# arpg/Kangaroo

Hardware: AMD Instinct MI355X
Metric: kinectfusion_frames_per_sec_640x480_to_512cubed_tsdf (higher is better)
Workload: dtype f32

## Files before the change

### include/kfx_debug.h

```cpp
#ifndef KFX_DEBUG_H
#define KFX_DEBUG_H

#include "kfx.h"

#ifdef __cplusplus
extern "C" {
#endif

int kfx_debug_rmw(const kfx_volume* vol, int variant, kfx_stream stream);

int kfx_debug_div_uniform_check(float b, unsigned long long* d_out, kfx_stream stream);

int kfx_debug_div_core_check(unsigned seed, int per_divisor, unsigned long long* d_out, kfx_stream stream);
int kfx_debug_sqrt_core_check(unsigned long long* d_out, kfx_stream stream);
int kfx_debug_wave_xor_check(unsigned seed, unsigned long long* d_out, kfx_stream stream);

int kfx_debug_summary_export(kfx_sdf_summary* s, float tol, float vref, int fine_shift, void* R_out, void* C_out, int dims_out[12],
                             kfx_stream stream);

int kfx_debug_summary_conditional_builds(kfx_sdf_summary* s, int out[2], kfx_stream stream);

int kfx_debug_summary_top_levels(kfx_sdf_summary* s, int fine_shift, void* top_out, int dims_out[12], unsigned long long* launches_out,
                                 kfx_stream stream);

int kfx_debug_fuse_keep(const kfx_sdf_summary* s, int out[3], unsigned char* kept, int n_rows);

#ifdef __cplusplus
}
#endif
#endif
```

### kangaroo_amd/csrc/raycast.hip

```cpp
#include <cmath>
#include <thread>

#include <hip/hip_fp16.h>

#include "kfx_device.h"
#include "sampling.h"
#include "raycast_ray.h"
#include "../../include/kfx_slab_color.h"

namespace kfx {

template <typename CELL, bool COLOR>
__device__ __forceinline__ void write_ray(const RayParams& q, const ColorGeom& cv, const int u, const int v, const float depth)
{
    const auto gradient_at = [&q](const V3 pos_w) { return gradient<CELL>(q, pos_w); };
    if constexpr (COLOR) write_ray(q, u, v, depth, gradient_at, [&cv](const V3 pos_w) { return trilinear<RayC32>(cv, pos_w); });
    else write_ray(q, u, v, depth, gradient_at, PhongShade{});
}

__device__ __forceinline__ unsigned touch(unsigned* bitmap, const VolView& v, int x, int y, int z)
{
    const size_t i = ((size_t)z * v.h + y) * v.w + x;
    const unsigned bit = 1u << (i & 31);
    unsigned* word = bitmap + (i >> 5);
    if (*reinterpret_cast<volatile unsigned*>(word) & bit) return 0u;
    return (atomicOr(word, bit) & bit) ? 0u : 1u;
}
__device__ __forceinline__ void touch_sample(unsigned* bitmap, const VolView& vol, const CellPos c, unsigned* cnt)
{
    cnt[0] += 1;
    for (int k = 0; k < 8; ++k) cnt[3] += touch(bitmap, vol, c.ix + (k & 1), c.iy + ((k >> 1) & 1), c.iz + (k >> 2));
}
__device__ __forceinline__ void touch_gradient(unsigned* bitmap, const RayParams& p, const V3 pos_w, unsigned* cnt)
{
    cnt[2] += 1;
    const CellPos b = gradient_base(p, pos_w);
    for (int dz = -1; dz < 2; ++dz)
        for (int dy = -1; dy < 2; ++dy)
            for (int dx = -1; dx < 2; ++dx)
                if ((dx < 0) + (dy < 0) + (dz < 0) <= 1) cnt[3] += touch(bitmap, p.vol, b.ix + dx, b.iy + dy, b.iz + dz);
}
// ... 12 lines not shown
}

template <typename CELL, bool COLOR, bool COUNT = false>
__device__ __forceinline__ float raycast_pixel(const RayParams& p, const ColorGeom& cv, const int u, const int v, unsigned* bitmap = nullptr,
                                               unsigned* cnt = nullptr)
{
    if (u >= p.w || v >= p.h) return 0.f;

    const RayBox box = ray_box(p, u, v);
    float depth = 0.0f;
    if (enters(box))
        depth = march_plain(p, box, [=](const RayParams& q, const V3 pos_w) {
            if constexpr (COUNT) touch_sample(bitmap, q.vol, cell_of(q, pos_w), cnt);
            return trilinear<CELL>(q, pos_w);
        });

    if constexpr (COUNT) {
        if (depth > 0) touch_gradient(bitmap, p, box.c_w + box.ray_w * depth, cnt);
    } else {
        write_ray<CELL, COLOR>(p, cv, u, v, depth);
    }
    return depth > 0 ? depth : __builtin_nanf("");
}

struct TopLevels { ClassLevel lv[2]; int n; };

__device__ __forceinline__ int class_lookup(const unsigned* tab, const ClassLevel& L, int gx, int gy, int gz)
{
    const int bx = gx >> L.shift, by = gy >> L.shift, bz = gz >> L.shift;
    const uint2 w = *reinterpret_cast<const uint2*>(tab + L.first + (bz * L.ny + by) * L.rw + ((bx >> 5) << 1));
    return (int)((w.x >> (bx & 31)) & 1u) | (int)(((w.y >> (bx & 31)) & 1u) << 1);
}

template <typename CELL, bool COLOR, bool COUNT = false, bool GT = false>
__device__ __forceinline__ float raycast_pixel_classes(const RayParams& p, const RayParams& q, const ColorGeom& cv, const int u, const int v, const ClassView& cl_arg, const unsigned* tab,
                                                       const TopLevels& top, unsigned* bitmap = nullptr, unsigned* cnt = nullptr)
{
    constexpr bool PARK = !GT && !COUNT;
    ClassView parked;
    if constexpr (PARK) parked = cl_arg;
    ClassView& clp = parked;
    if constexpr (PARK) {
        clp.fine.shift = in_vgpr(clp.fine.shift); clp.fine.ny = in_vgpr(clp.fine.ny); clp.fine.rw = in_vgpr(clp.fine.rw); clp.fine.first = in_vgpr(clp.fine.first);
        clp.coarse.ny = in_vgpr(clp.coarse.ny); clp.coarse.rw = in_vgpr(clp.coarse.rw); clp.coarse.first = in_vgpr(clp.coarse.first);
        clp.ox = in_vgpr(clp.ox); clp.oy = in_vgpr(clp.oy); clp.oz = in_vgpr(clp.oz);
        clp.eps = in_vgpr(clp.eps); clp.vref = in_vgpr(clp.vref);
    }
    const ClassView& cl = PARK ? parked : cl_arg;
    if (u >= p.w || v >= p.h) return 0.f;

    const RayBox box = ray_box(p, u, v);
    const V3 c_w = box.c_w, ray_w = box.ray_w;
    const float max_tmin = box.max_tmin, min_tmax = box.min_tmax;

    float depth = 0.0f;
    if (max_tmin < min_tmax) {
        float lambda = max_tmin;
        float last_sdf = __builtin_nanf("");
        const float min_delta = p.voxel.x;
        float delta = 0.f;
        const V3 sc = v3(p.dims1.x / p.size.x, p.dims1.y / p.size.y, p.dims1.z / p.size.z);
        const V3 pfA = v3((c_w.x - p.vol.bmin.x) * sc.x, (c_w.y - p.vol.bmin.y) * sc.y, (c_w.z - p.vol.bmin.z) * sc.z);
        const V3 pfB = v3(ray_w.x * sc.x, ray_w.y * sc.y, ray_w.z * sc.z);
        const V3 inv = v3(1.0f / pfB.x, 1.0f / pfB.y, 1.0f / pfB.z);
        const float eps = cl.eps;
        const float step_free = fmaxf(cl.vref, min_delta);
        const float inv_step_free = 1.0f / step_free, inv_trunc = 1.0f / p.trunc;
        const float band = cl.tol * cl.vref;
        bool pending = false;
        float lambda_prev = 0.f;
        bool consult = true;
        float lam_retry = lambda;
        int wait = 0, backoff = 1;
        while (lambda < min_tmax) {
            const bool look = consult && wait == 0 && lambda >= lam_retry;
            CellPos c{};
            typename CELL::InFlight fl;
            if (!look) {
                c = cell_of(p, c_w + ray_w * lambda);
                trilinear_issue<CELL>(fl, p, c);
                if constexpr (COUNT) touch_sample(bitmap, p.vol, c, cnt);
            }
            if (look) {
                if constexpr (COUNT) cnt[1] += 1;
                const float ex = __builtin_fmaf(pfB.x, lambda, pfA.x), ey = __builtin_fmaf(pfB.y, lambda, pfA.y), ez = __builtin_fmaf(pfB.z, lambda, pfA.z);
                const float flx = floorf(ex), fly = floorf(ey), flz = floorf(ez);
                const float lo_f = fminf(fminf(ex - flx, ey - fly), ez - flz), hi_f = fmaxf(fmaxf(ex - flx, ey - fly), ez - flz);
                bool run = false;
                if (fminf(fminf(ex, ey), ez) > eps && ex < p.dims1.x - eps && ey < p.dims1.y - eps && ez < p.dims1.z - eps && lo_f > eps && hi_f < 1.0f - eps) {
                    const int gx = (int)flx + cl.ox, gy = (int)fly + cl.oy, gz = (int)flz + cl.oz;
                    int cls = 0, shift = cl.fine.shift;
                    if constexpr (GT) {
                        if (cl.top_n > 1) {
                            int c7 = class_lookup(tab, top.lv[1], gx, gy, gz);
                            if (c7 == 3 && !cl.amb_ok) c7 = 0;
                            if (c7 != 0) { cls = c7; shift = 7; }
                        }
                        if (cls == 0 && cl.top_n > 0) {
                            int c6 = class_lookup(tab, top.lv[0], gx, gy, gz);
                            if (c6 == 3 && !cl.amb_ok) c6 = 0;
                            if (c6 != 0) { cls = c6; shift = 6; }
                        }
                        if (cls == 0) {
                            int c5 = class_lookup(cl.C, cl.coarse, gx, gy, gz);
                            if (c5 == 3 && !cl.amb_ok) c5 = 0;
                            if (c5 != 0) { cls = c5; shift = 5; }
                        }
                        if (cls == 0) {
// ... 46 lines not shown
                        backoff = 1;
                        run = true;
                    } else {
                        lam_retry = lam_exit;
                    }
                }
                if (!run) {
                    wait = backoff;
                    backoff = min(backoff * 2, 32);
                }
            }
            if (!look) {
                const float sdf = trilinear_finish<CELL>(fl, c);
                wait = max(wait - 1, 0);
                if (sdf <= 0) {
                    if (pending) {
                        last_sdf = trilinear<CELL>(p, c_w + ray_w * lambda_prev);
                        if constexpr (COUNT) touch_sample(bitmap, p.vol, cell_of(p, c_w + ray_w * lambda_prev), cnt);
                    }
                    if (last_sdf > 0) {
                        if (p.subpix) lambda = lambda + delta * sdf / (last_sdf - sdf);
                        depth = lambda;
                    }
                    break;
                }
                delta = march_step(sdf, min_delta, p.trunc);
                lambda += delta;
                last_sdf = sdf;
                pending = false;
                consult = !(fabsf(sdf - cl.vref) > band);
            }
        }
    }

    if constexpr (COUNT) {
        if (depth > 0) touch_gradient(bitmap, p, c_w + ray_w * depth, cnt);
    } else {
        write_ray<CELL, COLOR>(q, cv, u, v, depth);
    }
    return depth > 0 ? depth : __builtin_nanf("");
}

template <bool GT = false>
__device__ __forceinline__ void classes_stage(const ClassView& cl, unsigned* tab, TopLevels& top)
{
    const uint4* src = reinterpret_cast<const uint4*>(cl.C + (GT ? cl.top_first : 0));
    uint4* dst = reinterpret_cast<uint4*>(tab);
    for (int i = threadIdx.x; i < (cl.lds_words >> 2); i += blockDim.x) dst[i] = src[i];
    ClassLevel l6, l7;
    int nx6, nz6, nx7, nz7, w6, w7;
    const int at = GT ? 0 : cl.words;
    class_level_up(cl.nx5, cl.coarse.ny, cl.nz5, 6, at, l6, nx6, nz6, w6);
    class_level_up(nx6, l6.ny, nz6, 7, at + w6, l7, nx7, nz7, w7);
    if (threadIdx.x == 0) { top.lv[0] = l6; top.lv[1] = l7; top.n = cl.top_n; }
    __syncthreads();
}

__device__ __forceinline__ bool workgroup_any(const bool yes, int* s_any)
{
    const bool wave_any = __ballot(yes) != 0ull;
    if ((threadIdx.x & 63) == 0) s_any[threadIdx.x >> 6] = wave_any ? 1 : 0;
    __syncthreads();
    return (s_any[0] | s_any[1] | s_any[2] | s_any[3]) != 0;
}

template <typename CELL, bool GT = false>
__global__ __launch_bounds__(256) void k_raycast_sdf_classes(const RayParams p, const ClassView cl)
{
    extern __shared__ unsigned s_tab[];
    __shared__ RayParams s_p;
    __shared__ TopLevels s_top;
    __shared__ int s_any[4];
    if (threadIdx.x == 0) s_p = p;
    int u, v;
    const bool carries = ray_lane_pixel(p, p.sparse_lanes, blockIdx.x, blockIdx.y, u, v);
    const bool pixel = carries && u < p.w && v < p.h;
    if constexpr (!GT) {
        if (!workgroup_any(pixel && enters(ray_box(p, u, v)), s_any)) {
            if (pixel) write_no_hit(ray_out(p, u, v));
            return;
        }
    }
    classes_stage<GT>(cl, s_tab, s_top);
    if (!carries) return;
    raycast_pixel_classes<CELL, false, false, GT>(p, s_p, ColorGeom{}, u, v, cl, s_tab, s_top);
}

template <typename CELL, bool COLOR>
__global__ __launch_bounds__(256) void k_raycast_sdf(const RayParams p, const ColorGeom cv)
{
    int u, v;
    if (!ray_lane_pixel(p, p.sparse_lanes, blockIdx.x, blockIdx.y, u, v)) return;
    raycast_pixel<CELL, COLOR>(p, cv, u, v);
}

template <typename CELL>
__global__ __launch_bounds__(256) void k_raycast_sdf_count(const RayParams p, unsigned* __restrict__ bitmap, unsigned long long* __restrict__ counters)
{
    int u, v;
    ray_pixel_of(p, blockIdx.x, blockIdx.y, threadIdx.x, u, v);
    unsigned cnt[4] = {0u, 0u, 0u, 0u}, entered = 0;
    if (u < p.w && v < p.h) {
        entered = enters(ray_box(p, u, v)) ? 1u : 0u;
        raycast_pixel<CELL, false, true>(p, ColorGeom{}, u, v, bitmap, cnt);
    }
    publish_counts(cnt, entered, counters);
}

template <typename CELL, bool GT = false>
__global__ __launch_bounds__(256) void k_raycast_sdf_classes_count(const RayParams p, const ClassView cl, unsigned* __restrict__ bitmap,
                                                                   unsigned long long* __restrict__ counters)
{
    extern __shared__ unsigned s_tab[];
    __shared__ RayParams s_p;
    __shared__ TopLevels s_top;
    if (threadIdx.x == 0) s_p = p;
    classes_stage<GT>(cl, s_tab, s_top);
    int u, v;
    ray_pixel_of(p, blockIdx.x, blockIdx.y, threadIdx.x, u, v);
// ... 348 lines not shown
    cl.vref = vref;
    cl.amb_ok = fmaxf(vref, p.voxel.x) == p.trunc ? 1 : 0;
    cl.tol = tol;
    const double u24 = 1.0 / 16777216.0;
    double eps = 0.0;
    const float bmin[3] = {p.vol.bmin.x, p.vol.bmin.y, p.vol.bmin.z}, bmax[3] = {p.vol.bmax.x, p.vol.bmax.y, p.vol.bmax.z};
    const float size[3] = {p.size.x, p.size.y, p.size.z}, dims1[3] = {p.dims1.x, p.dims1.y, p.dims1.z};
    const float cw[3] = {p.T.m[3], p.T.m[7], p.T.m[11]};
    for (int a = 0; a < 3; ++a) {
        if (!(size[a] > 0.f)) return 0;
        const double sc = (double)dims1[a] / size[a];
        const double pmax = std::fmax(std::fabs((double)bmin[a]), std::fabs((double)bmax[a])), ca = std::fabs((double)cw[a]);
        const double A = std::fabs(((double)cw[a] - bmin[a]) * sc);
        const double t = sc * (3.0 * pmax + 2.0 * ca + size[a]) * u24 + 2.0 * dims1[a] * u24;
        const double e = u24 * (3.0 * A + 2.0 * sc * (pmax + ca) + dims1[a]) + 3.0 * u24 * (dims1[a] + A);
        eps = std::fmax(eps, t + e);
    }
    eps *= 2.0;
    if (!(eps < 0.05)) return 0;
    cl.eps = (float)std::fmax(eps, 1e-4);
    *lds_bytes = (size_t)cl.lds_words * sizeof(unsigned);
    *usable = 1;
    return 0;
}

template <typename PLAIN, typename... A>
static int launch_march(const char* what, int usable, const ClassView& cl, size_t cl_bytes, dim3 grid, kfx_stream stream, const RayParams& p,
                        void (*global)(RayParams, ClassView, A...), void (*lds)(RayParams, ClassView, A...), PLAIN plain, A... a)
{
    if (usable) hipLaunchKernelGGL(cl.global ? global : lds, grid, dim3(256), cl_bytes, (hipStream_t)stream, p, cl, a...);
    else plain();
    return check_launch(what);
}

template <typename CELL>
static int raycast_levels_launch(int n_levels, const kfx_image* const* depth, const kfx_image* const* norm, const kfx_image* const* img,
                                 const kfx_image* const* vbo, const kfx_volume* vol, const float T_wc[12], const float* K, float near, float far,
                                 float trunc_dist, int subpix, kfx_stream stream, kfx_sdf_summary* summary = nullptr)
{
    if (n_levels < 0 || n_levels > RAY_MAX_LEVELS) return set_error(KFX_E_RANGE, "RaycastSdf(levels): number of levels");
    if (!depth || !norm || !img || !K) return set_error(KFX_E_NULL, "RaycastSdf(levels): null argument");
    RayParams base{};
    RayLevels L{};
    int blocks = 0;
    for (int l = 0; l < n_levels; ++l) {
        RayParams p;
        if (int e = ray_params<CELL>(p, depth[l], norm[l], img[l], vol, T_wc, K + 4 * l, near, far, trunc_dist, subpix)) return e;
        if (p.w == 0 || p.h == 0) continue;
        RayLevel& lv = L.lv[L.n++];
        lv.dptr = p.dptr; lv.nptr = p.nptr; lv.iptr = p.iptr;
        lv.dpitch = p.dpitch; lv.npitch = p.npitch; lv.ipitch = p.ipitch;
        lv.w = p.w; lv.h = p.h;
        lv.K = p.K;
        lv.vptr = nullptr;
        lv.vpitch = 0;
        if (vbo && vbo[l]) {
            const kfx_image* vb = vbo[l];
            if (int e = check_image(vb, 16, (size_t)p.w, (size_t)p.h, "RaycastSdf(levels): vertex map")) return e;
            lv.vptr = (unsigned char*)vb->ptr;
            lv.vpitch = vb->pitch;
        }
        lv.first_block = blocks;
        static const int sparse_env = [] { const int v = env_int("KFX_RAYCAST_SPARSE", 16); return (v == 8 || v == 16 || v == 32) ? v : 0; }();
        lv.sparse = (long long)p.w * p.h <= 160 * 120 ? sparse_env : 0;
        lv.blocks_x = lv.sparse ? ceil_div(p.w, 2 * lv.sparse) : ceil_div(p.w, 64);
        blocks += lv.blocks_x * (lv.sparse ? ceil_div(p.h, 2) : ceil_div(p.h, 4));
// ... 9 lines not shown
        if (int e = class_view<CELL>(cl, &cl_bytes, &usable, summary, vol, base, stream, false)) return e;
        if (usable) {
            hipLaunchKernelGGL((k_raycast_sdf_levels_classes<CELL>), dim3(blocks), dim3(256), cl_bytes, (hipStream_t)stream, base, L, cl);
            return check_launch("kfx_raycast_sdf_levels_tracked");
        }
    }
    hipLaunchKernelGGL((k_raycast_sdf_levels<CELL>), dim3(blocks), dim3(256), 0, (hipStream_t)stream, base, L);
    return check_launch("kfx_raycast_sdf_levels");
}

template <typename CELL>
static int raycast_launch(const kfx_image* depth, const kfx_image* norm, const kfx_image* img,
                          const kfx_volume* vol, const float T_wc[12], const float K[4], float near,
                          float far, float trunc_dist, int subpix, kfx_stream stream, const kfx_volume* colorvol = nullptr,
                          kfx_sdf_summary* summary = nullptr)
{
    RayParams p;
    if (int e = ray_params<CELL>(p, depth, norm, img, vol, T_wc, K, near, far, trunc_dist, subpix)) return e;
    if (summary && summary->cell_bytes != CELL::BYTES)
        return set_error(KFX_E_SHAPE, "RaycastSdf(tracked): the summary was created for the other cell type (kfx_sdf_summary_create / _create_h)");
    if (p.w == 0 || p.h == 0) return 0;

    const dim3 grid = ray_tiling(p);
    ColorGeom cv{};
    if (colorvol) {
        if (int e = check_volume(colorvol, 4, 2, VOLUME_ANY_DIM, "RaycastSdf(colour)")) return e;
        set_geometry(cv, colorvol);
        hipLaunchKernelGGL((k_raycast_sdf<CELL, true>), grid, dim3(256), 0, (hipStream_t)stream, p, cv);
    } else if (summary) {
        ClassView cl;
        size_t cl_bytes = 0;
        int usable = 0;
        if (int e = class_view<CELL>(cl, &cl_bytes, &usable, summary, vol, p, stream)) return e;
        return launch_march("kfx_raycast_sdf_tracked", usable, cl, cl_bytes, grid, stream, p, k_raycast_sdf_classes<CELL, true>, k_raycast_sdf_classes<CELL, false>,
                            [&] { hipLaunchKernelGGL((k_raycast_sdf<CELL, false>), grid, dim3(256), 0, (hipStream_t)stream, p, cv); });
    } else {
        hipLaunchKernelGGL((k_raycast_sdf<CELL, false>), grid, dim3(256), 0, (hipStream_t)stream, p, cv);
    }
    return check_launch("kfx_raycast_sdf");
}

extern "C" int kfx_raycast_sdf(const kfx_image* depth, const kfx_image* norm, const kfx_image* img,
                               const kfx_volume* vol, const float T_wc[12], const float K[4], float near,
                               float far, float trunc_dist, int subpix, kfx_stream stream)
{
    return raycast_launch<RayF32>(depth, norm, img, vol, T_wc, K, near, far, trunc_dist, subpix, stream);
}

template <typename CELL>
static int count_params(RayParams& p, dim3& grid, const kfx_volume* vol, unsigned w, unsigned h, const float T_wc[12], const float K[4], float near, float far,
                        float trunc_dist, int subpix)
{
    kfx_image dummy = {(size_t)w * 16, (void*)(uintptr_t)16, w, h};
    if (int e = ray_params<CELL>(p, &dummy, &dummy, &dummy, vol, T_wc, K, near, far, trunc_dist, subpix)) return e;
    p.dptr = p.nptr = p.iptr = nullptr;
    grid = pixel_grid(p.w, p.h);
    return 0;
}

template <typename CELL>
static int raycast_count_launch(const kfx_volume* vol, unsigned w, unsigned h, const float T_wc[12], const float K[4], float near, float far,
                                float trunc_dist, int subpix, unsigned* d_bitmap, unsigned long long* d_counters, kfx_stream stream)
{
    if (!d_bitmap || !d_counters) return set_error(KFX_E_NULL, "kfx_raycast_sdf_count: null argument");
    RayParams p;
    dim3 grid;
    if (int e = count_params<CELL>(p, grid, vol, w, h, T_wc, K, near, far, trunc_dist, subpix)) return e;
    if (p.w == 0 || p.h == 0) return 0;
// ... 27 lines not shown
    if (p.w == 0 || p.h == 0) return 0;
    ClassView cl;
    size_t cl_bytes = 0;
    int usable = 0;
    const unsigned plain_calls = summary->plain_calls;
    const int ce = class_view<CELL>(cl, &cl_bytes, &usable, summary, vol, p, stream);
    summary->plain_calls = plain_calls;
    if (ce) return ce;
    return launch_march("kfx_raycast_sdf_count_tracked", usable, cl, cl_bytes, grid, stream, p, k_raycast_sdf_classes_count<CELL, true>,
                        k_raycast_sdf_classes_count<CELL, false>,
                        [&] { hipLaunchKernelGGL(k_raycast_sdf_count<CELL>, grid, dim3(256), 0, (hipStream_t)stream, p, d_bitmap, d_counters); }, d_bitmap, d_counters);
}

extern "C" int kfx_raycast_sdf_count_tracked(const kfx_volume* vol, kfx_sdf_summary* summary, unsigned w, unsigned h, const float T_wc[12], const float K[4],
                                             float near, float far, float trunc_dist, int subpix, unsigned* d_bitmap, unsigned long long* d_counters,
                                             kfx_stream stream)
{
    return raycast_count_tracked_launch<RayF32>(vol, summary, w, h, T_wc, K, near, far, trunc_dist, subpix, d_bitmap, d_counters, stream);
}

extern "C" int kfx_raycast_sdf_count_tracked_h(const kfx_volume* vol, kfx_sdf_summary* summary, unsigned w, unsigned h, const float T_wc[12], const float K[4],
                                               float near, float far, float trunc_dist, int subpix, unsigned* d_bitmap, unsigned long long* d_counters,
                                               kfx_stream stream)
{
    return raycast_count_tracked_launch<RayF16>(vol, summary, w, h, T_wc, K, near, far, trunc_dist, subpix, d_bitmap, d_counters, stream);
}

extern "C" int kfx_raycast_sdf_tracked(const kfx_image* depth, const kfx_image* norm, const kfx_image* img, const kfx_volume* vol,
                                       kfx_sdf_summary* summary, const float T_wc[12], const float K[4], float near, float far,
                                       float trunc_dist, int subpix, kfx_stream stream)
{
    if (!summary) return set_error(KFX_E_NULL, "kfx_raycast_sdf_tracked: null summary");
    return raycast_launch<RayF32>(depth, norm, img, vol, T_wc, K, near, far, trunc_dist, subpix, stream, nullptr, summary);
}

extern "C" int kfx_raycast_sdf_tracked_h(const kfx_image* depth, const kfx_image* norm, const kfx_image* img, const kfx_volume* vol,
                                         kfx_sdf_summary* summary, const float T_wc[12], const float K[4], float near, float far,
                                         float trunc_dist, int subpix, kfx_stream stream)
{
    if (!summary) return set_error(KFX_E_NULL, "kfx_raycast_sdf_tracked_h: null summary");
    return raycast_launch<RayF16>(depth, norm, img, vol, T_wc, K, near, far, trunc_dist, subpix, stream, nullptr, summary);
}

extern "C" int kfx_raycast_sdf_h(const kfx_image* depth, const kfx_image* norm, const kfx_image* img,
                                 const kfx_volume* vol, const float T_wc[12], const float K[4], float near,
                                 float far, float trunc_dist, int subpix, kfx_stream stream)
{
    return raycast_launch<RayF16>(depth, norm, img, vol, T_wc, K, near, far, trunc_dist, subpix, stream);
}

extern "C" int kfx_raycast_sdf_levels(int n_levels, const kfx_image* const* depth, const kfx_image* const* norm, const kfx_image* const* img,
                                      const kfx_image* const* vbo, const kfx_volume* vol, const float T_wc[12], const float* K, float near, float far,
                                      float trunc_dist, int subpix, kfx_stream stream)
{
    return raycast_levels_launch<RayF32>(n_levels, depth, norm, img, vbo, vol, T_wc, K, near, far, trunc_dist, subpix, stream);
}

extern "C" int kfx_raycast_sdf_levels_tracked(int n_levels, const kfx_image* const* depth, const kfx_image* const* norm, const kfx_image* const* img,
                                              const kfx_image* const* vbo, const kfx_volume* vol, kfx_sdf_summary* summary, const float T_wc[12],
                                              const float* K, float near, float far, float trunc_dist, int subpix, kfx_stream stream)
{
    if (!summary) return set_error(KFX_E_NULL, "kfx_raycast_sdf_levels_tracked: null summary");
    return raycast_levels_launch<RayF32>(n_levels, depth, norm, img, vbo, vol, T_wc, K, near, far, trunc_dist, subpix, stream, summary);
}

extern "C" int kfx_raycast_sdf_levels_h(int n_levels, const kfx_image* const* depth, const kfx_image* const* norm, const kfx_image* const* img,
// ... 162 lines not shown
    if (!colorvol) return set_error(KFX_E_NULL, "RaycastSdf(slab, colour): null colour volume");
    return raycast_slab_launch<RayF32>(dense_state(state, init, w, h), vol, slab, own_lo, own_hi, w, h, T_wc, K, near, far, trunc_dist, subpix, stream, colorvol);
}

extern "C" int kfx_raycast_sdf_slab(float* state, int init, const kfx_volume* vol, const kfx_slab* slab, int own_lo, int own_hi,
                                    int w, int h, const float T_wc[12], const float K[4], float near, float far,
                                    float trunc_dist, int subpix, kfx_stream stream)
{
    return raycast_slab_launch<RayF32>(dense_state(state, init, w, h), vol, slab, own_lo, own_hi, w, h, T_wc, K, near, far, trunc_dist, subpix, stream);
}

extern "C" int kfx_raycast_sdf_slab_h(float* state, int init, const kfx_volume* vol, const kfx_slab* slab, int own_lo, int own_hi,
                                      int w, int h, const float T_wc[12], const float K[4], float near, float far,
                                      float trunc_dist, int subpix, kfx_stream stream)
{
    return raycast_slab_launch<RayF16>(dense_state(state, init, w, h), vol, slab, own_lo, own_hi, w, h, T_wc, K, near, far, trunc_dist, subpix, stream);
}

extern "C" int kfx_raycast_state_to_images(const kfx_image* depth, const kfx_image* norm, const kfx_image* img, const float* state,
                                           kfx_stream stream)
{
    if (!state) return set_error(KFX_E_NULL, "raycast state: null argument");
    if (int e = check_image(img, 4, 0, 0, "raycast state")) return e;
    if (int e = check_image(depth, 4, cover_w(img), cover_h(img), "raycast state")) return e;
    if (int e = check_image(norm, 16, cover_w(img), cover_h(img), "raycast state")) return e;
    if (img->w == 0 || img->h == 0) return 0;
    RayParams p{};
    p.dptr = (unsigned char*)depth->ptr; p.nptr = (unsigned char*)norm->ptr; p.iptr = (unsigned char*)img->ptr;
    p.dpitch = depth->pitch; p.npitch = norm->pitch; p.ipitch = img->pitch;
    p.w = (int)img->w; p.h = (int)img->h;
    hipLaunchKernelGGL(k_raycast_state_to_images, pixel_grid(p.w, p.h), dim3(256), 0, (hipStream_t)stream, p, state);
    return check_launch("kfx_raycast_state_to_images");
}
```

### kangaroo_amd/csrc/raycast_ray.h

```cpp
#pragma once

#include <type_traits>

#include "kfx_device.h"
#include "sampling.h"

namespace kfx {

struct RayParams {
    VolView vol;
    V3 size;
    V3 dims1;
    V3 hi2;
    V3 voxel;
    V3 inv_size;
    int fastdiv, off32;
    Pose T;
    Intr K;
    unsigned char *dptr, *nptr, *iptr;
    size_t dpitch, npitch, ipitch;
    int w, h;
    float near, far, trunc;
    int subpix;
    int tile_log2w;
    int wg_log2x;
    int sparse_lanes;
};

__device__ __forceinline__ float phong(const V3 p_c, const V3 n_c)
{
    const float ambient = (float)0.4, diffuse = (float)0.4, specular = (float)0.2;
    const V3 eyedir = div_s(p_c * -1.0f, length(p_c));
    const V3 l0 = v3((float)0.4, (float)0.4, -1.0f);
    const V3 lightdir = div_s(l0, length(l0));
    const float ldotn = dot(lightdir, n_c);
    const V3 lightreflect = n_c * (2 * ldotn) + lightdir * -1.0f;
    const float edotr = fmaxf(0.0f, dot(eyedir, lightreflect));
    const float spec = edotr * edotr * edotr * edotr * edotr * edotr * edotr * edotr * edotr * edotr;
    return ambient + diffuse * ldotn + specular * spec;
}

__device__ __forceinline__ void ray_pixel_of(const RayParams& p, int bx, int by, int tid, int& u, int& v)
{
    const int lane = tid & 63, wv = tid >> 6;
    const int tw = 1 << p.tile_log2w, th = 64 >> p.tile_log2w;
    const int wgx = 1 << p.wg_log2x, wgy = 4 >> p.wg_log2x;
    u = (bx * wgx + (wv & (wgx - 1))) * tw + (lane & (tw - 1));
    v = (by * wgy + (wv >> p.wg_log2x)) * th + (lane >> p.tile_log2w);
}

__device__ __forceinline__ bool ray_lane_pixel(const RayParams& p, int sparse, int bx, int by, int& u, int& v)
{
    if (!sparse) {
        ray_pixel_of(p, bx, by, threadIdx.x, u, v);
        return true;
    }
    const int lane = threadIdx.x & 63, wv = threadIdx.x >> 6;
    u = (bx * 2 + (wv & 1)) * sparse + lane;
    v = by * 2 + (wv >> 1);
    return lane < sparse;
// ... 10 lines not shown
    const V3 tb = div_cw(p.vol.bmax - b.c_w, b.ray_w);
    const V3 tmin = v3(fminf(ta.x, tb.x), fminf(ta.y, tb.y), fminf(ta.z, tb.z));
    const V3 tmax = v3(fmaxf(ta.x, tb.x), fmaxf(ta.y, tb.y), fmaxf(ta.z, tb.z));
    b.max_tmin = fmaxf(fmaxf(fmaxf(tmin.x, tmin.y), tmin.z), p.near);
    b.min_tmax = fminf(fminf(fminf(tmax.x, tmax.y), tmax.z), p.far);
    return b;
}
__device__ __forceinline__ bool enters(const RayBox& b) { return b.max_tmin < b.min_tmax; }

__device__ __forceinline__ V3 normal_of(const Pose& T, const V3 g)
{
    const float len = length(g);
    const V3 n_w = len > 0 ? div_s(g, len) : v3(0.f, 0.f, 1.f);
    return so3_mul_inv(T, n_w);
}
template <typename CELL>
__device__ __forceinline__ V3 normal_c(const RayParams& p, const V3 pos_w)
{
    return normal_of(p.T, gradient<CELL>(p, pos_w));
}

struct RayOut { float* depth; float* shade; float4* normal; };
template <typename IMAGES>
__device__ __forceinline__ RayOut ray_out(const IMAGES& p, const int u, const int v)
{
    return RayOut{reinterpret_cast<float*>(p.dptr + (size_t)v * p.dpitch) + u, reinterpret_cast<float*>(p.iptr + (size_t)v * p.ipitch) + u,
                  reinterpret_cast<float4*>(p.nptr + (size_t)v * p.npitch) + u};
}
__device__ __forceinline__ void write_no_hit(const RayOut& o)
{
    *o.depth = __builtin_nanf("");
    *o.shade = 0.f;
    *o.normal = make_float4(0.f, 0.f, 0.f, 0.f);
}
__device__ __forceinline__ void write_hit(const RayOut& o, const float depth, const float4 normal, const float shade)
{
    *o.depth = depth;
    *o.shade = shade;
    *o.normal = normal;
}

template <typename PARAMS, typename SAMPLE>
__device__ __forceinline__ float march_plain(const PARAMS& p, const RayBox& box, const SAMPLE& sample)
{
    const V3 c_w = box.c_w, ray_w = box.ray_w;
    const float max_tmin = box.max_tmin, min_tmax = box.min_tmax;
    float depth = 0.0f;
    float lambda = max_tmin;
    float last_sdf = __builtin_nanf("");
    const float min_delta = p.voxel.x;
    float delta = 0.f;
    while (lambda < min_tmax) {
        const float sdf = sample(p, c_w + ray_w * lambda);
        if (sdf <= 0) {
            if (last_sdf > 0) {
                if (p.subpix) lambda = lambda + delta * sdf / (last_sdf - sdf);
                depth = lambda;
            }
            break;
        }
        delta = march_step(sdf, min_delta, p.trunc);
        lambda += delta;
        last_sdf = sdf;
    }
    return depth;
}
// ... 7 lines not shown
        const RayBox r = ray_box(q, u, v);
        const V3 n_c = normal_of(q.T, gradient_at(r.c_w + r.ray_w * depth));
        *o.depth = depth;
        if constexpr (std::is_same<SHADE, PhongShade>::value) *o.shade = phong(r.ray_c * depth, n_c);
        else *o.shade = shade(r.c_w + r.ray_w * depth);
        *o.normal = make_float4(n_c.x, n_c.y, n_c.z, 1.0f);
    } else {
        write_no_hit(o);
    }
}

inline void ray_fill(RayParams& p, const kfx_image* depth, const kfx_image* norm, const kfx_image* img, const float T_wc[12], const float K[4],
                     float near, float far, float trunc_dist, int subpix)
{
    for (int i = 0; i < 12; ++i) p.T.m[i] = T_wc[i];
    p.K = Intr{K[0], K[1], K[2], K[3]};
    p.dptr = (unsigned char*)depth->ptr;
    p.nptr = (unsigned char*)norm->ptr;
    p.iptr = (unsigned char*)img->ptr;
    p.dpitch = depth->pitch;
    p.npitch = norm->pitch;
    p.ipitch = img->pitch;
    p.w = (int)img->w;
    p.h = (int)img->h;
    p.near = near;
    p.far = far;
    p.trunc = trunc_dist;
    p.subpix = subpix ? 1 : 0;
    p.tile_log2w = 5;
    p.wg_log2x = 1;
    p.sparse_lanes = 0;
}

inline dim3 ray_tiling(RayParams& p)
{
    static const int tile_env = env_int("KFX_RAYCAST_TILE", 5, 0, 6);
    static const int wg_env = env_int("KFX_RAYCAST_WG", 1, 0, 2);
    static const int lanes_env = [] { const int v = env_int("KFX_RAYCAST_LANES", 0); return (v == 8 || v == 16 || v == 32) ? v : (v < 0 ? -1 : 0); }();
    p.tile_log2w = tile_env;
    p.wg_log2x = wg_env;
    const int lanes = lanes_env ? lanes_env : ((long long)p.w * p.h <= 160 * 120 ? 16 : 0);
    if (lanes && lanes_env >= 0) {
        p.sparse_lanes = lanes;
        return dim3(ceil_div(p.w, 2 * lanes), ceil_div(p.h, 2));
    }
    return dim3(ceil_div(p.w, (1 << p.wg_log2x) << p.tile_log2w), ceil_div(p.h, (4 >> p.wg_log2x) * (64 >> p.tile_log2w)));
}

}
```

Before: 2630.

## Plan raycast grid from projected volume rectangle and occupancy-based lane choice

Projects the volume's bounding box corners into the image on the host to find the pixel rectangle that can hit the volume. The class-table march then launches only over that rectangle, and extra block rows write no-hit outputs to the tiles outside it. The sparse lane count is chosen from the rectangle area and the measured wave capacity of the device instead of a fixed image-size rule. This adds host-side planning, an occupancy query cached per kernel, and a debug budget twin kernel, at the risk of less useful tiling when the camera sits inside the volume.

```diff
diff --git a/include/kfx_debug.h b/include/kfx_debug.h
--- a/include/kfx_debug.h
+++ b/include/kfx_debug.h
@@ -25,6 +25,10 @@
 
 int kfx_debug_fuse_keep(const kfx_sdf_summary* s, int out[3], unsigned char* kept, int n_rows);
 
+int kfx_debug_raycast_budget(const kfx_image* depth, const kfx_image* norm, const kfx_image* img, const kfx_volume* vol, kfx_sdf_summary* summary,
+                             const float T_wc[12], const float K[4], float near, float far, float trunc_dist, int subpix,
+                             unsigned long long* d_out, size_t out_words, int grid_out[3], kfx_stream stream);
+
 #ifdef __cplusplus
 }
 #endif
diff --git a/include/kfx_raycast_plan.h b/include/kfx_raycast_plan.h
--- /dev/null
+++ b/include/kfx_raycast_plan.h
@@ -0,0 +1,18 @@
+#ifndef KFX_RAYCAST_PLAN_H
+#define KFX_RAYCAST_PLAN_H
+
+#include "kfx.h"
+
+#ifdef __cplusplus
+extern "C" {
+#endif
+
+int kfx_raycast_plan(const float boxmin[3], const float boxmax[3], const float T_wc[12], const float K[4], float near, unsigned w, unsigned h,
+                     long long capacity_waves, long long out[10]);
+
+int kfx_raycast_last_plan(long long out[10]);
+
+#ifdef __cplusplus
+}
+#endif
+#endif
diff --git a/kangaroo_amd/csrc/raycast.hip b/kangaroo_amd/csrc/raycast.hip
--- a/kangaroo_amd/csrc/raycast.hip
+++ b/kangaroo_amd/csrc/raycast.hip
@@ -1,5 +1,7 @@
 #include <cmath>
+#include <mutex>
 #include <thread>
+#include <vector>
 
 #include <hip/hip_fp16.h>
 
@@ -7,6 +9,7 @@
 #include "sampling.h"
 #include "raycast_ray.h"
 #include "../../include/kfx_slab_color.h"
+#include "../../include/kfx_raycast_plan.h"
 
 namespace kfx {
 
@@ -85,9 +88,10 @@
     return (int)((w.x >> (bx & 31)) & 1u) | (int)(((w.y >> (bx & 31)) & 1u) << 1);
 }
 
-template <typename CELL, bool COLOR, bool COUNT = false, bool GT = false>
+template <typename CELL, bool COLOR, bool COUNT = false, bool GT = false, bool BUDGET = false>
 __device__ __forceinline__ float raycast_pixel_classes(const RayParams& p, const RayParams& q, const ColorGeom& cv, const int u, const int v, const ClassView& cl_arg, const unsigned* tab,
-                                                       const TopLevels& top, unsigned* bitmap = nullptr, unsigned* cnt = nullptr)
+                                                       const TopLevels& top, unsigned* bitmap = nullptr, unsigned* cnt = nullptr, unsigned* it = nullptr,
+                                                       unsigned long long* t_exit = nullptr)
 {
     constexpr bool PARK = !GT && !COUNT;
     ClassView parked;
@@ -127,6 +131,12 @@
         int wait = 0, backoff = 1;
         while (lambda < min_tmax) {
             const bool look = consult && wait == 0 && lambda >= lam_retry;
+            if constexpr (BUDGET) {
+                const bool looks = __ballot(look) != 0ull, samples = __ballot(!look) != 0ull;
+                it[0] += (looks && !samples) ? 1u : 0u;
+                it[1] += (!looks && samples) ? 1u : 0u;
+                it[2] += (looks && samples) ? 1u : 0u;
+            }
             CellPos c{};
             typename CELL::InFlight fl;
             if (!look) {
@@ -239,6 +249,7 @@
             }
         }
     }
+    if constexpr (BUDGET) *t_exit = wall_clock64();
 
     if constexpr (COUNT) {
         if (depth > 0) touch_gradient(bitmap, p, c_w + ray_w * depth, cnt);
@@ -272,15 +283,22 @@
 }
 
 template <typename CELL, bool GT = false>
-__global__ __launch_bounds__(256) void k_raycast_sdf_classes(const RayParams p, const ClassView cl)
+__global__ __launch_bounds__(256) void k_raycast_sdf_classes(const RayParams p, const ClassView cl, const RayRect rc)
 {
     extern __shared__ unsigned s_tab[];
     __shared__ RayParams s_p;
     __shared__ TopLevels s_top;
     __shared__ int s_any[4];
+    if constexpr (!GT) {
+        if ((int)blockIdx.y >= rc.march_rows) {
+            ray_fill_tile(p, rc, ((int)blockIdx.y - rc.march_rows) * (int)gridDim.x + (int)blockIdx.x);
+            return;
+        }
+    }
     if (threadIdx.x == 0) s_p = p;
     int u, v;
     const bool carries = ray_lane_pixel(p, p.sparse_lanes, blockIdx.x, blockIdx.y, u, v);
+    if constexpr (!GT) { u += rc.x0; v += rc.y0; }
     const bool pixel = carries && u < p.w && v < p.h;
     if constexpr (!GT) {
         if (!workgroup_any(pixel && enters(ray_box(p, u, v)), s_any)) {
@@ -292,6 +310,60 @@
     if (!carries) return;
     raycast_pixel_classes<CELL, false, false, GT>(p, s_p, ColorGeom{}, u, v, cl, s_tab, s_top);
 }
+
+#ifdef KFX_RAYCAST_BUDGET_TWIN
+template <typename CELL>
+__global__ __launch_bounds__(256) void k_raycast_sdf_classes_budget(const RayParams p, const ClassView cl, const RayRect rc, unsigned long long* __restrict__ out)
+{
+    extern __shared__ unsigned s_tab[];
+    __shared__ RayParams s_p;
+    __shared__ TopLevels s_top;
+    __shared__ int s_any[4];
+    const unsigned long long t_entry = wall_clock64();
+    unsigned long long* o = out + 8 * ((size_t)(blockIdx.y * gridDim.x + blockIdx.x) * 4 + (threadIdx.x >> 6));
+    const bool first = (threadIdx.x & 63) == 0;
+    const auto store = [&](unsigned long long t_vote, unsigned long long t_staged, unsigned long long t_exit, unsigned look, unsigned sample, unsigned mixed,
+                           unsigned rays, unsigned what) {
+        if (!first) return;
+        o[0] = t_entry; o[1] = t_vote; o[2] = t_staged; o[3] = t_exit; o[4] = wall_clock64();
+        o[5] = (unsigned long long)look | ((unsigned long long)sample << 32);
+        o[6] = (unsigned long long)mixed | ((unsigned long long)rays << 32);
+        o[7] = what;
+    };
+    if ((int)blockIdx.y >= rc.march_rows) {
+        ray_fill_tile(p, rc, ((int)blockIdx.y - rc.march_rows) * (int)gridDim.x + (int)blockIdx.x);
+        store(0, 0, 0, 0, 0, 0, 0, 0);
+        return;
+    }
+    if (threadIdx.x == 0) s_p = p;
+    int u, v;
+    const bool carries = ray_lane_pixel(p, p.sparse_lanes, blockIdx.x, blockIdx.y, u, v);
+    u += rc.x0; v += rc.y0;
+    const bool pixel = carries && u < p.w && v < p.h;
+    const bool in_box = pixel && enters(ray_box(p, u, v));
+    const unsigned rays = (unsigned)__popcll(__ballot(in_box));
+    const bool any = workgroup_any(in_box, s_any);
+    const unsigned long long t_vote = wall_clock64();
+    if (!any) {
+        if (pixel) write_no_hit(ray_out(p, u, v));
+        store(t_vote, 0, 0, 0, 0, 0, rays, 1);
+        return;
+    }
+    classes_stage<false>(cl, s_tab, s_top);
+    const unsigned long long t_staged = wall_clock64();
+    unsigned it[3] = {0u, 0u, 0u};
+    unsigned long long t_exit = 0;
+    if (carries) raycast_pixel_classes<CELL, false, false, false, true>(p, s_p, ColorGeom{}, u, v, cl, s_tab, s_top, nullptr, nullptr, it, &t_exit);
+#pragma unroll
+    for (int off = 32; off > 0; off >>= 1) {
+#pragma unroll
+        for (int k = 0; k < 3; ++k) it[k] = max(it[k], (unsigned)__shfl_xor((int)it[k], off, 64));
+        const unsigned long long other = ((unsigned long long)(unsigned)__shfl_xor((int)(t_exit >> 32), off, 64) << 32) | (unsigned)__shfl_xor((int)(unsigned)t_exit, off, 64);
+        t_exit = other > t_exit ? other : t_exit;
+    }
+    store(t_vote, t_staged, t_exit, it[0], it[1], it[2], rays, 2);
+}
+#endif
 
 template <typename CELL, bool COLOR>
 __global__ __launch_bounds__(256) void k_raycast_sdf(const RayParams p, const ColorGeom cv)
@@ -706,6 +778,74 @@
     else plain();
     return check_launch(what);
 }
+
+static int wave_capacity(const void* kernel, const size_t lds_bytes, long long* waves)
+{
+    struct Entry { const void* kernel; size_t lds; int device; long long waves; };
+    static std::mutex mu;
+    static std::vector<Entry> known;
+    int device = 0;
+    if (int e = hip_status(hipGetDevice(&device), "RaycastSdf(tracked): hipGetDevice")) return e;
+    std::lock_guard<std::mutex> lock(mu);
+    for (const Entry& e : known)
+        if (e.kernel == kernel && e.lds == lds_bytes && e.device == device) { *waves = e.waves; return 0; }
+    int blocks = 0, cus = 0;
+    if (int e = hip_status(hipOccupancyMaxActiveBlocksPerMultiprocessor(&blocks, kernel, 256, lds_bytes), "RaycastSdf(tracked): occupancy of the class-table march")) return e;
+    if (int e = hip_status(hipDeviceGetAttribute(&cus, hipDeviceAttributeMultiprocessorCount, device), "RaycastSdf(tracked): compute units of the device")) return e;
+    if (blocks < 1 || cus < 1) return set_error(KFX_E_RANGE, "RaycastSdf(tracked): the class-table march does not fit a compute unit");
+    known.push_back(Entry{kernel, lds_bytes, device, (long long)blocks * 4 * cus});
+    *waves = known.back().waves;
+    return 0;
+}
+
+static void plan_out(long long out[10], const RayPlan& plan, const int rule, const int launched, const long long capacity, const long long launches)
+{
+    const long long v[10] = {plan.x0, plan.y0, plan.x1, plan.y1, plan.bound, plan.whole, rule, launched, capacity, launches};
+    for (int k = 0; k < 10; ++k) out[k] = v[k];
+}
+static thread_local long long t_last_plan[10] = {0, 0, 0, 0, 0, 0, 0, 0, 0, 0};
+
+static int planned_tiling(dim3& grid, RayRect& rc, RayParams& p, const void* kernel, const size_t lds_bytes, const bool rect)
+{
+    long long capacity = 0;
+    if (int e = wave_capacity(kernel, lds_bytes, &capacity)) return e;
+    const RayPlan plan = ray_plan(p);
+    const int rule = ray_plan_lanes(plan.bound, capacity);
+    grid = ray_tiling(p, rule);
+    rc = RayRect{0, 0, (int)grid.y, 0, 0, 0, 0, 0, 0};
+    if (rect) grid = ray_rect_grid(rc, p, plan, grid);
+    plan_out(t_last_plan, plan, rule, p.sparse_lanes ? p.sparse_lanes : 64, capacity, t_last_plan[9] + 1);
+    return 0;
+}
+
+#ifdef KFX_RAYCAST_BUDGET_TWIN
+static int raycast_budget_launch(const kfx_image* depth, const kfx_image* norm, const kfx_image* img, const kfx_volume* vol, kfx_sdf_summary* summary,
+                          const float T_wc[12], const float K[4], float near, float far, float trunc_dist, int subpix, unsigned long long* d_out,
+                          size_t out_words, int grid_out[3], kfx_stream stream)
+{
+    if (!summary || !grid_out) return set_error(KFX_E_NULL, "kfx_debug_raycast_budget: null argument");
+    RayParams p;
+    if (int e = ray_params<RayF32>(p, depth, norm, img, vol, T_wc, K, near, far, trunc_dist, subpix)) return e;
+    if (summary->cell_bytes != RayF32::BYTES) return set_error(KFX_E_SHAPE, "kfx_debug_raycast_budget: the summary was created for the other cell type");
+    if (p.w == 0 || p.h == 0) return set_error(KFX_E_SHAPE, "kfx_debug_raycast_budget: empty image");
+    ClassView cl;
+    size_t cl_bytes = 0;
+    int usable = 0;
+    const unsigned plain_calls = summary->plain_calls;
+    const int ce = class_view<RayF32>(cl, &cl_bytes, &usable, summary, vol, p, stream);
+    summary->plain_calls = plain_calls;
+    if (ce) return ce;
+    if (!usable || cl.global) return set_error(KFX_E_RANGE, "kfx_debug_raycast_budget: the tracked call would not run the LDS-mode table march here");
+    dim3 grid;
+    RayRect rc{};
+    if (int e = planned_tiling(grid, rc, p, (const void*)k_raycast_sdf_classes<RayF32, false>, cl_bytes, true)) return e;
+    grid_out[0] = (int)grid.x; grid_out[1] = (int)grid.y; grid_out[2] = (int)(grid.x * grid.y * 4);
+    if (!d_out) return 0;
+    if (out_words < (size_t)grid.x * grid.y * 4 * 8) return set_error(KFX_E_SHAPE, "kfx_debug_raycast_budget: eight words per wave of the grid");
+    hipLaunchKernelGGL(k_raycast_sdf_classes_budget<RayF32>, grid, dim3(256), cl_bytes, (hipStream_t)stream, p, cl, rc, d_out);
+    return check_launch("kfx_debug_raycast_budget");
+}
+#else
 
 template <typename CELL>
 static int raycast_levels_launch(int n_levels, const kfx_image* const* depth, const kfx_image* const* norm, const kfx_image* const* img,
@@ -781,8 +921,14 @@
         size_t cl_bytes = 0;
         int usable = 0;
         if (int e = class_view<CELL>(cl, &cl_bytes, &usable, summary, vol, p, stream)) return e;
-        return launch_march("kfx_raycast_sdf_tracked", usable, cl, cl_bytes, grid, stream, p, k_raycast_sdf_classes<CELL, true>, k_raycast_sdf_classes<CELL, false>,
-                            [&] { hipLaunchKernelGGL((k_raycast_sdf<CELL, false>), grid, dim3(256), 0, (hipStream_t)stream, p, cv); });
+        dim3 march_grid = grid;
+        RayRect rc{};
+        if (usable) {
+            const void* kernel = cl.global ? (const void*)k_raycast_sdf_classes<CELL, true> : (const void*)k_raycast_sdf_classes<CELL, false>;
+            if (int e = planned_tiling(march_grid, rc, p, kernel, cl_bytes, !cl.global)) return e;
+        }
+        return launch_march("kfx_raycast_sdf_tracked", usable, cl, cl_bytes, march_grid, stream, p, k_raycast_sdf_classes<CELL, true>, k_raycast_sdf_classes<CELL, false>,
+                            [&] { hipLaunchKernelGGL((k_raycast_sdf<CELL, false>), grid, dim3(256), 0, (hipStream_t)stream, p, cv); }, rc);
     } else {
         hipLaunchKernelGGL((k_raycast_sdf<CELL, false>), grid, dim3(256), 0, (hipStream_t)stream, p, cv);
     }
@@ -876,6 +1022,33 @@
 {
     if (!summary) return set_error(KFX_E_NULL, "kfx_raycast_sdf_tracked: null summary");
     return raycast_launch<RayF32>(depth, norm, img, vol, T_wc, K, near, far, trunc_dist, subpix, stream, nullptr, summary);
+}
+
+extern "C" int kfx_raycast_plan(const float boxmin[3], const float boxmax[3], const float T_wc[12], const float K[4], float near, unsigned w, unsigned h,
+                                long long capacity_waves, long long out[10])
+{
+    if (!boxmin || !boxmax || !T_wc || !K || !out) return set_error(KFX_E_NULL, "kfx_raycast_plan: null argument");
+    if (w > 0x7fffffffu || h > 0x7fffffffu) return set_error(KFX_E_RANGE, "kfx_raycast_plan: image dimensions");
+    RayParams p{};
+    p.vol.bmin = V3{boxmin[0], boxmin[1], boxmin[2]};
+    p.vol.bmax = V3{boxmax[0], boxmax[1], boxmax[2]};
+    for (int i = 0; i < 12; ++i) p.T.m[i] = T_wc[i];
+    p.K = Intr{K[0], K[1], K[2], K[3]};
+    p.near = near;
+    p.w = (int)w;
+    p.h = (int)h;
+    const RayPlan plan = ray_plan(p);
+    const int rule = capacity_waves > 0 ? ray_plan_lanes(plan.bound, capacity_waves) : 0;
+    plan_out(out, plan, rule, rule, capacity_waves > 0 ? capacity_waves : 0, 0);
+    return 0;
+}
+
+extern "C" int kfx_raycast_last_plan(long long out[10])
+{
+    if (!out) return set_error(KFX_E_NULL, "kfx_raycast_last_plan: null argument");
+    if (t_last_plan[9] == 0) return set_error(KFX_E_RANGE, "kfx_raycast_last_plan: this thread has launched no class-table march");
+    for (int k = 0; k < 10; ++k) out[k] = t_last_plan[k];
+    return 0;
 }
 
 extern "C" int kfx_raycast_sdf_tracked_h(const kfx_image* depth, const kfx_image* norm, const kfx_image* img, const kfx_volume* vol,
@@ -1104,3 +1277,4 @@
     hipLaunchKernelGGL(k_raycast_state_to_images, pixel_grid(p.w, p.h), dim3(256), 0, (hipStream_t)stream, p, state);
     return check_launch("kfx_raycast_state_to_images");
 }
+#endif
diff --git a/kangaroo_amd/csrc/raycast_budget.hip b/kangaroo_amd/csrc/raycast_budget.hip
--- /dev/null
+++ b/kangaroo_amd/csrc/raycast_budget.hip
@@ -0,0 +1,10 @@
+#define KFX_RAYCAST_BUDGET_TWIN 1
+#include "raycast.hip"
+#include "../../include/kfx_debug.h"
+
+extern "C" int kfx_debug_raycast_budget(const kfx_image* depth, const kfx_image* norm, const kfx_image* img, const kfx_volume* vol, kfx_sdf_summary* summary,
+                                        const float T_wc[12], const float K[4], float near, float far, float trunc_dist, int subpix,
+                                        unsigned long long* d_out, size_t out_words, int grid_out[3], kfx_stream stream)
+{
+    return raycast_budget_launch(depth, norm, img, vol, summary, T_wc, K, near, far, trunc_dist, subpix, d_out, out_words, grid_out, stream);
+}
diff --git a/kangaroo_amd/csrc/raycast_ray.h b/kangaroo_amd/csrc/raycast_ray.h
--- a/kangaroo_amd/csrc/raycast_ray.h
+++ b/kangaroo_amd/csrc/raycast_ray.h
@@ -1,5 +1,7 @@
 #pragma once
 
+#include <algorithm>
+#include <cmath>
 #include <type_traits>
 
 #include "kfx_device.h"
@@ -26,6 +28,10 @@
     int wg_log2x;
     int sparse_lanes;
 };
+struct RayRect {
+    int x0, y0, march_rows;
+    int fill_n, fill_tx, fill_rx0, fill_rx1, fill_ry0, fill_ry1;
+};
 
 __device__ __forceinline__ float phong(const V3 p_c, const V3 n_c)
 {
@@ -102,6 +108,24 @@
     *o.depth = __builtin_nanf("");
     *o.shade = 0.f;
     *o.normal = make_float4(0.f, 0.f, 0.f, 0.f);
+}
+__device__ __forceinline__ void ray_fill_tile(const RayParams& p, const RayRect& r, const int idx)
+{
+    if (idx >= r.fill_n) return;
+    const int gap = r.fill_rx1 - r.fill_rx0, beside = r.fill_tx - gap;
+    const int above = r.fill_ry0 * r.fill_tx, sides = (r.fill_ry1 - r.fill_ry0) * beside;
+    int tx, ty;
+    if (idx < above) {
+        ty = idx / r.fill_tx; tx = idx - ty * r.fill_tx;
+    } else if (idx < above + sides) {
+        const int j = idx - above, row = j / beside, k = j - row * beside;
+        ty = r.fill_ry0 + row; tx = k < r.fill_rx0 ? k : k + gap;
+    } else {
+        const int j = idx - above - sides, row = j / r.fill_tx;
+        ty = r.fill_ry1 + row; tx = j - row * r.fill_tx;
+    }
+    const int u = tx * PIX_W + (int)(threadIdx.x & 63), v = ty * PIX_H + (int)(threadIdx.x >> 6);
+    if (u < p.w && v < p.h) write_no_hit(ray_out(p, u, v));
 }
 __device__ __forceinline__ void write_hit(const RayOut& o, const float depth, const float4 normal, const float shade)
 {
@@ -175,19 +199,72 @@
     p.sparse_lanes = 0;
 }
 
-inline dim3 ray_tiling(RayParams& p)
+struct RayPlan { int x0, y0, x1, y1; long long bound; int whole; };
+inline RayPlan ray_plan(const RayParams& p)
+{
+    const RayPlan all{0, 0, p.w, p.h, (long long)p.w * p.h, 1};
+    const double c[3] = {p.T.m[3], p.T.m[7], p.T.m[11]};
+    const double lo[3] = {p.vol.bmin.x, p.vol.bmin.y, p.vol.bmin.z}, hi[3] = {p.vol.bmax.x, p.vol.bmax.y, p.vol.bmax.z};
+    if (c[0] >= lo[0] && c[0] <= hi[0] && c[1] >= lo[1] && c[1] <= hi[1] && c[2] >= lo[2] && c[2] <= hi[2]) return all;
+    double umin = 1e300, umax = -1e300, vmin = 1e300, vmax = -1e300;
+    for (int k = 0; k < 8; ++k) {
+        const double d[3] = {((k & 1) ? hi[0] : lo[0]) - c[0], ((k & 2) ? hi[1] : lo[1]) - c[1], ((k & 4) ? hi[2] : lo[2]) - c[2]};
+        const double X = p.T.m[0] * d[0] + p.T.m[4] * d[1] + p.T.m[8] * d[2], Y = p.T.m[1] * d[0] + p.T.m[5] * d[1] + p.T.m[9] * d[2],
+                     Z = p.T.m[2] * d[0] + p.T.m[6] * d[1] + p.T.m[10] * d[2];
+        if (!(Z > (double)p.near) || !(Z > 0.0)) return all;
+        const double u = (double)p.K.fu * X / Z + p.K.u0, v = (double)p.K.fv * Y / Z + p.K.v0;
+        if (!(std::fabs(u) < 1e9) || !(std::fabs(v) < 1e9)) return all;
+        umin = std::fmin(umin, u); umax = std::fmax(umax, u); vmin = std::fmin(vmin, v); vmax = std::fmax(vmax, v);
+    }
+    RayPlan r;
+    r.x0 = (int)std::fmax(std::floor(umin) - 1.0, 0.0);
+    r.y0 = (int)std::fmax(std::floor(vmin) - 1.0, 0.0);
+    r.x1 = (int)std::fmin(std::ceil(umax) + 2.0, (double)p.w);
+    r.y1 = (int)std::fmin(std::ceil(vmax) + 2.0, (double)p.h);
+    r.whole = 0;
+    if (r.x1 <= r.x0 || r.y1 <= r.y0) r = RayPlan{0, 0, 0, 0, 0, 0};
+    r.bound = (long long)(r.x1 - r.x0) * (r.y1 - r.y0);
+    return r;
+}
+inline int ray_plan_lanes(const long long bound, const long long capacity_waves)
+{
+    for (int rays = 16; rays < 64; rays *= 2)
+        if ((bound + rays - 1) / rays <= capacity_waves) return rays;
+    return 64;
+}
+
+inline int ray_block_w(const RayParams& p) { return p.sparse_lanes ? 2 * p.sparse_lanes : (1 << p.wg_log2x) << p.tile_log2w; }
+inline int ray_block_h(const RayParams& p) { return p.sparse_lanes ? 2 : (4 >> p.wg_log2x) * (64 >> p.tile_log2w); }
+
+inline dim3 ray_tiling(RayParams& p, const int planned = 0)
 {
     static const int tile_env = env_int("KFX_RAYCAST_TILE", 5, 0, 6);
     static const int wg_env = env_int("KFX_RAYCAST_WG", 1, 0, 2);
     static const int lanes_env = [] { const int v = env_int("KFX_RAYCAST_LANES", 0); return (v == 8 || v == 16 || v == 32) ? v : (v < 0 ? -1 : 0); }();
     p.tile_log2w = tile_env;
     p.wg_log2x = wg_env;
-    const int lanes = lanes_env ? lanes_env : ((long long)p.w * p.h <= 160 * 120 ? 16 : 0);
-    if (lanes && lanes_env >= 0) {
-        p.sparse_lanes = lanes;
-        return dim3(ceil_div(p.w, 2 * lanes), ceil_div(p.h, 2));
-    }
-    return dim3(ceil_div(p.w, (1 << p.wg_log2x) << p.tile_log2w), ceil_div(p.h, (4 >> p.wg_log2x) * (64 >> p.tile_log2w)));
-}
-
-}
+    p.sparse_lanes = 0;
+    const int rule = planned ? (planned < 64 ? planned : 0) : ((long long)p.w * p.h <= 160 * 120 ? 16 : 0);
+    const int lanes = lanes_env ? lanes_env : rule;
+    if (lanes && lanes_env >= 0) p.sparse_lanes = lanes;
+    return dim3(ceil_div(p.w, ray_block_w(p)), ceil_div(p.h, ray_block_h(p)));
+}
+
+inline dim3 ray_rect_grid(RayRect& r, const RayParams& p, const RayPlan& plan, const dim3 whole)
+{
+    static const int rect_env = env_int("KFX_RAYCAST_RECT", 1);
+    const int bw = ray_block_w(p), bh = ray_block_h(p);
+    r = RayRect{0, 0, (int)whole.y, 0, 0, 0, 0, 0, 0};
+    if (!rect_env || plan.whole || PIX_W % bw || PIX_H % bh) return whole;
+    const int tx = ceil_div(p.w, PIX_W), ty = ceil_div(p.h, PIX_H);
+    const int rx0 = plan.x0 / PIX_W, rx1 = ceil_div(plan.x1, PIX_W), ry0 = plan.y0 / PIX_H, ry1 = ceil_div(plan.y1, PIX_H);
+    const long long fill = (long long)tx * ty - (long long)(rx1 - rx0) * (ry1 - ry0);
+    const int gx = rx1 > rx0 ? ceil_div(std::min(rx1 * PIX_W, p.w) - rx0 * PIX_W, bw) : tx;
+    const int rows = rx1 > rx0 ? ceil_div(std::min(ry1 * PIX_H, p.h) - ry0 * PIX_H, bh) : 0;
+    const long long fill_rows = (fill + gx - 1) / gx;
+    if (rows + fill_rows > 65535) return whole;
+    r = RayRect{rx0 * PIX_W, ry0 * PIX_H, rows, (int)fill, tx, rx0, rx1, ry0, ry1};
+    return dim3(gx, rows + (int)fill_rows);
+}
+
+}
```

New measurement: 2627. Within noise of the previous version (-0.1%).
